# CloudEngineHub/FairyGen

Hardware: AMD Instinct MI355X
Metric: decoded frames/sec (sec/clip in config), Wan2.2-TI2V-5B 704x1280x121 @ 5 steps (higher is better)
Workload: dtype bf16

## Files before the change

### fairygen_amd/csrc/dit_elementwise.hip

```cpp
#include "common.h"
#include "rmsnorm_rope_row.h"

#ifndef FG_ROW_MIN_WAVES
#define FG_ROW_MIN_WAVES 4
#endif
#define FG_ROW_BOUNDS __launch_bounds__(256, FG_ROW_MIN_WAVES)

namespace {

__device__ __forceinline__ void row_moments(const Row& r, int C, int lane, float eps, float& mean, float& rstd) {
    const int nvec = C >> 3;
    float s = 0.f;
#pragma unroll
    for (int i = 0; i < kMaxVec; ++i)
#pragma unroll
        for (int j = 0; j < 8; ++j) s += r.v[i][j];
    mean = wave_sum(s) / (float)C;
    float q = 0.f;
#pragma unroll
    for (int i = 0; i < kMaxVec; ++i) {
        if (lane + i * 64 < nvec) {
#pragma unroll
            for (int j = 0; j < 8; ++j) {
                const float d = r.v[i][j] - mean;
                q += d * d;
            }
        }
    }
    const float var = wave_sum(q) / (float)C;
    rstd = 1.0f / sqrtf(var + eps);
}

__device__ __forceinline__ int64_t mod_row(int64_t row, int64_t mod_rows, int64_t first_rows) {
    return mod_rows == 1 ? 0 : (mod_rows == 2 ? (row < first_rows ? 0 : 1) : row);
}

template <int MODE>
__device__ __forceinline__ void norm_store(const Row& r, int C, int lane, float eps, const bf16* p0, const bf16* p1,
                                           bf16* out) {
    const int nvec = C >> 3;
    float mean, rstd;
    row_moments(r, C, lane, eps, mean, rstd);
#pragma unroll
    for (int i = 0; i < kMaxVec; ++i) {
        const int vi = lane + i * 64;
        if (vi < nvec) {
            const bf16x8 a = ld8(p0 + (int64_t)vi * 8);
            const bf16x8 b = ld8(p1 + (int64_t)vi * 8);
            float o[8];
#pragma unroll
            for (int j = 0; j < 8; ++j) {
                const float n = (r.v[i][j] - mean) * rstd;
                if (MODE == 0) {
                    const float y = rbf(n);
                    const float s1 = rbf(1.0f + (float)b[j]);
                    o[j] = rbf(y * s1) + (float)a[j];
                } else {
                    o[j] = n * (float)a[j] + (float)b[j];
                }
            }
            st8(out + (int64_t)vi * 8, o);
        }
    }
}

__device__ __forceinline__ uint32_t cvt2_fp8(float a, float b) {
    return (uint32_t)__builtin_amdgcn_cvt_pk_fp8_f32(a, b, 0, false) & 0xffffu;
}

template <int MODE, bool DUAL = false>
__device__ __forceinline__ void norm_store_fp8(Row& r, int C, int lane, float eps, const bf16* p0, const bf16* p1,
                                               uint8_t* out8, float* scale_out, float fp8_max, bf16* out16 = nullptr) {
    const int nvec = C >> 3;
    float mean, rstd;
    row_moments(r, C, lane, eps, mean, rstd);
    float amax = 0.f;
#pragma unroll
    for (int i = 0; i < kMaxVec; ++i) {
        const int vi = lane + i * 64;
        if (vi < nvec) {
            const bf16x8 a = ld8(p0 + (int64_t)vi * 8);
            const bf16x8 b = ld8(p1 + (int64_t)vi * 8);
#pragma unroll
            for (int j = 0; j < 8; ++j) {
                const float n = (r.v[i][j] - mean) * rstd;
                float o;
                if (MODE == 0) {
                    const float y = rbf(n);
                    const float s1 = rbf(1.0f + (float)b[j]);
                    o = rbf(y * s1) + (float)a[j];
                } else {
                    o = n * (float)a[j] + (float)b[j];
                }
                r.v[i][j] = rbf(o);
                amax = fmaxf(amax, fabsf(r.v[i][j]));
            }
            if (DUAL) st8(out16 + (int64_t)vi * 8, r.v[i]);
        }
    }
    amax = wave_max(amax);
    const float sc = fmaxf(rbf(amax / fp8_max), 1.0f);
    const float denom = sc + 1e-8f;
    if (lane == 0) *scale_out = sc;
#pragma unroll
    for (int i = 0; i < kMaxVec; ++i) {
        const int vi = lane + i * 64;
        if (vi < nvec) {
            u32x2 w;
            w[0] = cvt2_fp8(r.v[i][0] / denom, r.v[i][1] / denom) | (cvt2_fp8(r.v[i][2] / denom, r.v[i][3] / denom) << 16);
            w[1] = cvt2_fp8(r.v[i][4] / denom, r.v[i][5] / denom) | (cvt2_fp8(r.v[i][6] / denom, r.v[i][7] / denom) << 16);
            *reinterpret_cast<u32x2*>(out8 + (int64_t)vi * 8) = w;
        }
    }
}

__global__ FG_ROW_BOUNDS void ln_modulate_fp8_kernel(const bf16* __restrict__ x, const bf16* __restrict__ shift,
                                                     const bf16* __restrict__ scale, uint8_t* __restrict__ out8,
                                                     float* __restrict__ scale_out, int64_t rows, int C, float eps, int64_t mod_rows,
                                                     int64_t first_rows, int64_t mod_ld, float fp8_max) {
    const int lane = threadIdx.x & 63;
    const int64_t row = (int64_t)blockIdx.x * kRowsPerBlock + (threadIdx.x >> 6);
    if (row >= rows) return;
    Row r;
    load_row(x + row * C, C, lane, r);
    const int64_t m = mod_row(row, mod_rows, first_rows);
    norm_store_fp8<0>(r, C, lane, eps, shift + m * mod_ld, scale + m * mod_ld, out8 + row * C, scale_out + row, fp8_max);
}

template <int MODE>
__global__ FG_ROW_BOUNDS void ln_dual_kernel(const bf16* __restrict__ x, const bf16* __restrict__ p0, const bf16* __restrict__ p1,
                                             bf16* __restrict__ out, uint8_t* __restrict__ out8, float* __restrict__ scale_out,
                                             int64_t rows, int C, float eps, int64_t mod_rows, int64_t first_rows, int64_t mod_ld,
                                             float fp8_max) {
    const int lane = threadIdx.x & 63;
    const int64_t row = (int64_t)blockIdx.x * kRowsPerBlock + (threadIdx.x >> 6);
    if (row >= rows) return;
    Row r;
    load_row(x + row * C, C, lane, r);
    const int64_t m = MODE == 0 ? mod_row(row, mod_rows, first_rows) : 0;
    norm_store_fp8<MODE, true>(r, C, lane, eps, p0 + m * mod_ld, p1 + m * mod_ld, out8 + row * C, scale_out + row, fp8_max, out + row * C);
}

__global__ FG_ROW_BOUNDS void ln_modulate_kernel(const bf16* __restrict__ x, const bf16* __restrict__ shift,
                                                          const bf16* __restrict__ scale, bf16* __restrict__ out,
                                                          int64_t rows, int C, float eps, int64_t mod_rows,
                                                          int64_t first_rows, int64_t mod_ld) {
    const int lane = threadIdx.x & 63;
    const int64_t row = (int64_t)blockIdx.x * kRowsPerBlock + (threadIdx.x >> 6);
    if (row >= rows) return;
    Row r;
    load_row(x + row * C, C, lane, r);
    const int64_t m = mod_row(row, mod_rows, first_rows);
    norm_store<0>(r, C, lane, eps, shift + m * mod_ld, scale + m * mod_ld, out + row * C);
}

__global__ FG_ROW_BOUNDS void ln_affine_kernel(const bf16* __restrict__ x, const bf16* __restrict__ w,
                                                        const bf16* __restrict__ b, bf16* __restrict__ out,
                                                        int64_t rows, int C, float eps) {
    const int lane = threadIdx.x & 63;
    const int64_t row = (int64_t)blockIdx.x * kRowsPerBlock + (threadIdx.x >> 6);
    if (row >= rows) return;
    Row r;
    load_row(x + row * C, C, lane, r);
    norm_store<1>(r, C, lane, eps, w, b, out + row * C);
}

template <int MODE>
__global__ FG_ROW_BOUNDS void residual_kernel(const bf16* __restrict__ x, const bf16* __restrict__ y,
                                                       const bf16* __restrict__ gate, bf16* __restrict__ x_out,
                                                       const bf16* __restrict__ p0, const bf16* __restrict__ p1,
                                                       bf16* __restrict__ norm_out, int64_t rows, int C, float eps,
                                                       int64_t mod_rows, int64_t first_rows, int64_t mod_ld,
                                                       uint8_t* __restrict__ norm_fp8 = nullptr, float* __restrict__ norm_scale = nullptr,
                                                       float fp8_max = 0.f) {
    const int lane = threadIdx.x & 63;
    const int64_t row = (int64_t)blockIdx.x * kRowsPerBlock + (threadIdx.x >> 6);
    if (row >= rows) return;
    const int nvec = C >> 3;
    const int64_t m = mod_row(row, mod_rows, first_rows);
    Row r;
#pragma unroll
    for (int i = 0; i < kMaxVec; ++i) {
        const int vi = lane + i * 64;
        if (vi < nvec) {
            const bf16x8 xv = ld8(x + row * C + (int64_t)vi * 8);
            const bf16x8 yv = ld8(y + row * C + (int64_t)vi * 8);
            if (gate != nullptr) {
                const bf16x8 gv = ld8(gate + m * mod_ld + (int64_t)vi * 8);
#pragma unroll
                for (int j = 0; j < 8; ++j) r.v[i][j] = rbf((float)xv[j] + rbf((float)gv[j] * (float)yv[j]));
            } else {
#pragma unroll
                for (int j = 0; j < 8; ++j) r.v[i][j] = rbf((float)xv[j] + (float)yv[j]);
            }
            st8(x_out + row * C + (int64_t)vi * 8, r.v[i]);
        } else {
#pragma unroll
            for (int j = 0; j < 8; ++j) r.v[i][j] = 0.f;
        }
    }
    if (norm_fp8 != nullptr) {
        if (MODE == 0) norm_store_fp8<0>(r, C, lane, eps, p0 + m * mod_ld, p1 + m * mod_ld, norm_fp8 + row * C, norm_scale + row, fp8_max);
        if (MODE == 1) norm_store_fp8<1>(r, C, lane, eps, p0, p1, norm_fp8 + row * C, norm_scale + row, fp8_max);
        return;
    }
    if (MODE == 0) norm_store<0>(r, C, lane, eps, p0 + m * mod_ld, p1 + m * mod_ld, norm_out + row * C);
    if (MODE == 1) norm_store<1>(r, C, lane, eps, p0, p1, norm_out + row * C);
}

template <bool F32TAB, bool PLAIN = false>
__global__ FG_ROW_BOUNDS void rmsnorm_rope_kernel(const bf16* __restrict__ x, int64_t ldx,
                                                           const bf16* __restrict__ w, const void* __restrict__ ctv,
                                                           const void* __restrict__ stv, bf16* __restrict__ out,
                                                           int64_t rows, int C, int head_dim, float eps, int group_cols,
                                                           int64_t out_group_stride, int64_t out_ld) {
    const int lane = threadIdx.x & 63;
    const int64_t row = (int64_t)blockIdx.x * kRowsPerBlock + (threadIdx.x >> 6);
    if (row >= rows) return;
    Row r;
    load_row(x + row * ldx, C, lane, r);
    const int nvec = C >> 3;
    const RopeRow rr = rope_begin<F32TAB, PLAIN>(r, ctv, row, C, head_dim, eps, lane);
#pragma unroll
    for (int i = 0; i < kMaxVec; ++i) {
        const int vi = lane + i * 64;
        if (vi < nvec) {
            float o[8];
            rope_vec<F32TAB, PLAIN>(rr, r.v[i], ld8(w + (int64_t)vi * 8), ctv, stv, row, head_dim, vi, o);
            const int col = vi * 8, g = PLAIN ? 0 : col / group_cols;
            st8(out + g * out_group_stride + row * out_ld + (col - g * group_cols), o);
        }
    }
}

__global__ __launch_bounds__(256) void copy_groups_kernel(const bf16* __restrict__ src, int64_t sgs, int64_t sld,
                                                          bf16* __restrict__ dst, int64_t dgs, int64_t dld, int groups,
                                                          int64_t rows, int vec_per_row) {
    const int64_t total = (int64_t)groups * rows * vec_per_row;
    for (int64_t i = (int64_t)blockIdx.x * blockDim.x + threadIdx.x; i < total; i += (int64_t)gridDim.x * blockDim.x) {
        const int64_t rg = i / vec_per_row;
        const int v = (int)(i - rg * vec_per_row);
        const int64_t r = rg / groups;
        const int g = (int)(rg - r * groups);
        *reinterpret_cast<u32x4*>(dst + g * dgs + r * dld + v * 8) =
            *reinterpret_cast<const u32x4*>(src + g * sgs + r * sld + v * 8);
    }
}


template <int KIND>
__global__ __launch_bounds__(256) void act_kernel(const bf16* __restrict__ x, bf16* __restrict__ out, int64_t nvec) {
    for (int64_t i = (int64_t)blockIdx.x * blockDim.x + threadIdx.x; i < nvec; i += (int64_t)gridDim.x * blockDim.x) {
        const bf16x8 v = ld8(x + i * 8);
        float o[8];
#pragma unroll
        for (int j = 0; j < 8; ++j) o[j] = KIND == 0 ? silu_f((float)v[j]) : gelu_tanh_f((float)v[j]);
        st8(out + i * 8, o);
    }
}

__device__ __forceinline__ float cfg_euler_one(float lat, float p, float ng, bool has_nega, float cfg, float dsigma) {
    const float pred = has_nega ? rbf(ng + rbf(cfg * rbf(p - ng))) : p;
    return rbf(lat + rbf(pred * dsigma));
}

__global__ __launch_bounds__(256) void cfg_euler_kernel(const bf16* __restrict__ lat, const bf16* __restrict__ posi,
                                                        const bf16* __restrict__ nega, bf16* __restrict__ out,
                                                        int64_t n, float cfg, float dsigma) {
    for (int64_t i = (int64_t)blockIdx.x * blockDim.x + threadIdx.x; i < n; i += (int64_t)gridDim.x * blockDim.x)
        out[i] = (bf16)cfg_euler_one((float)lat[i], (float)posi[i], nega != nullptr ? (float)nega[i] : 0.0f, nega != nullptr, cfg, dsigma);
}

__global__ __launch_bounds__(256) void cfg_euler_dev_kernel(const bf16* lat, const bf16* __restrict__ posi, const bf16* __restrict__ nega,
                                                            bf16* out, int64_t n, int64_t nvec, float cfg,
                                                            const float* __restrict__ dsigma_table, const int* __restrict__ step,
                                                            const bf16* __restrict__ first, int64_t first_n, int64_t frame_stride) {
    const float dsigma = dsigma_table[*step];
    const bool has_nega = nega != nullptr;
    const int64_t tid = (int64_t)blockIdx.x * blockDim.x + threadIdx.x, nthreads = (int64_t)gridDim.x * blockDim.x;
    for (int64_t i = tid; i < nvec; i += nthreads) {
        const bf16x8 l = ld8(lat + i * 8), p = ld8(posi + i * 8);
        const bf16x8 g = has_nega ? ld8(nega + i * 8) : p;
        float o[8];
#pragma unroll
        for (int j = 0; j < 8; ++j) o[j] = cfg_euler_one((float)l[j], (float)p[j], (float)g[j], has_nega, cfg, dsigma);
        if (first != nullptr) {
            int64_t ch = (i * 8) / frame_stride, r = i * 8 - ch * frame_stride;
            if (r < first_n || r + 7 >= frame_stride) {
#pragma unroll
                for (int j = 0; j < 8; ++j) {
                    if (r < first_n) o[j] = (float)first[ch * first_n + r];
                    if (++r == frame_stride) { r = 0; ++ch; }
                }
            }
        }
        st8(out + i * 8, o);
    }
    for (int64_t i = nvec * 8 + tid; i < n; i += nthreads) {
        float o = cfg_euler_one((float)lat[i], (float)posi[i], has_nega ? (float)nega[i] : 0.0f, has_nega, cfg, dsigma);
        if (first != nullptr) {
            const int64_t ch = i / frame_stride, r = i - ch * frame_stride;
            if (r < first_n) o = (float)first[ch * first_n + r];
        }
        out[i] = (bf16)o;
    }
}

inline int check_rows(const char* fn, int64_t rows, int C, int64_t mod_rows, int64_t first_rows) {
    FG_CHECK_ARG(rows >= 0 && C > 0 && (C % 8) == 0 && C <= kMaxVec * 512, "%s: need C %% 8 == 0 and C <= %d (got rows=%lld C=%d)",
                 fn, kMaxVec * 512, (long long)rows, C);
    FG_CHECK_ARG(mod_rows == 1 || mod_rows == 2 || mod_rows == rows, "%s: mod_rows must be 1, 2 or rows (got %lld)", fn,
                 (long long)mod_rows);
    FG_CHECK_ARG(first_rows >= 0 && first_rows <= rows, "%s: first_rows out of range", fn);
    return FG_OK;
}

inline dim3 row_grid(int64_t rows) { return dim3((unsigned)((rows + kRowsPerBlock - 1) / kRowsPerBlock)); }

}

extern "C" {

int fg_ln_modulate_bf16(const void* x, const void* shift, const void* scale, void* out, int64_t rows, int C, float eps,
                        int64_t mod_rows, int64_t first_rows, int64_t mod_ld, fg_stream_t stream) {
    if (int e = check_rows("fg_ln_modulate_bf16", rows, C, mod_rows, first_rows)) return e;
    FG_CHECK_ARG(x && shift && scale && out, "fg_ln_modulate_bf16: null pointer");
    FG_CHECK_ARG(FG_ALIGNED16(x) && FG_ALIGNED16(shift) && FG_ALIGNED16(scale) && FG_ALIGNED16(out) && mod_ld % 8 == 0,
                 "fg_ln_modulate_bf16: pointers / mod_ld must be 16-byte aligned");
    if (rows == 0) return FG_OK;
    hipLaunchKernelGGL(ln_modulate_kernel, row_grid(rows), dim3(256), 0, (hipStream_t)stream, (const bf16*)x,
                       (const bf16*)shift, (const bf16*)scale, (bf16*)out, rows, C, eps, mod_rows, first_rows, mod_ld);
    return fg_launch_status("fg_ln_modulate_bf16");
}

int fg_ln_modulate_fp8_bf16(const void* x, const void* shift, const void* scale, void* out_fp8, float* out_scale, int64_t rows, int C,
                            float eps, int64_t mod_rows, int64_t first_rows, int64_t mod_ld, float fp8_max, fg_stream_t stream) {
    if (int e = check_rows("fg_ln_modulate_fp8_bf16", rows, C, mod_rows, first_rows)) return e;
    FG_CHECK_ARG(x && shift && scale && out_fp8 && out_scale, "fg_ln_modulate_fp8_bf16: null pointer");
    FG_CHECK_ARG(FG_ALIGNED16(x) && FG_ALIGNED16(shift) && FG_ALIGNED16(scale) && (((uintptr_t)out_fp8) & 7) == 0 && mod_ld % 8 == 0 &&
                     fp8_max > 0.f,
                 "fg_ln_modulate_fp8_bf16: pointers / mod_ld must be 16-byte aligned (out_fp8: 8), fp8_max positive");
    if (rows == 0) return FG_OK;
    hipLaunchKernelGGL(ln_modulate_fp8_kernel, row_grid(rows), dim3(256), 0, (hipStream_t)stream, (const bf16*)x, (const bf16*)shift,
                       (const bf16*)scale, (uint8_t*)out_fp8, out_scale, rows, C, eps, mod_rows, first_rows, mod_ld, fp8_max);
    return fg_launch_status("fg_ln_modulate_fp8_bf16");
}

int fg_ln_modulate_dual_bf16(const void* x, const void* shift, const void* scale, void* out, void* out_fp8, float* out_scale,
                             int64_t rows, int C, float eps, int64_t mod_rows, int64_t first_rows, int64_t mod_ld, float fp8_max,
                             fg_stream_t stream) {
    if (int e = check_rows("fg_ln_modulate_dual_bf16", rows, C, mod_rows, first_rows)) return e;
    FG_CHECK_ARG(x && shift && scale && out && out_fp8 && out_scale, "fg_ln_modulate_dual_bf16: null pointer");
    FG_CHECK_ARG(FG_ALIGNED16(x) && FG_ALIGNED16(shift) && FG_ALIGNED16(scale) && FG_ALIGNED16(out) && (((uintptr_t)out_fp8) & 7) == 0 &&
                     mod_ld % 8 == 0 && fp8_max > 0.f,
                 "fg_ln_modulate_dual_bf16: pointers / mod_ld must be 16-byte aligned (out_fp8: 8), fp8_max positive");
    if (rows == 0) return FG_OK;
    hipLaunchKernelGGL(ln_dual_kernel<0>, row_grid(rows), dim3(256), 0, (hipStream_t)stream, (const bf16*)x, (const bf16*)shift,
                       (const bf16*)scale, (bf16*)out, (uint8_t*)out_fp8, out_scale, rows, C, eps, mod_rows, first_rows, mod_ld, fp8_max);
    return fg_launch_status("fg_ln_modulate_dual_bf16");
}

int fg_ln_affine_dual_bf16(const void* x, const void* w, const void* b, void* out, void* out_fp8, float* out_scale, int64_t rows, int C,
                           float eps, float fp8_max, fg_stream_t stream) {
    if (int e = check_rows("fg_ln_affine_dual_bf16", rows, C, 1, 0)) return e;
    FG_CHECK_ARG(x && w && b && out && out_fp8 && out_scale, "fg_ln_affine_dual_bf16: null pointer");
    FG_CHECK_ARG(FG_ALIGNED16(x) && FG_ALIGNED16(w) && FG_ALIGNED16(b) && FG_ALIGNED16(out) && (((uintptr_t)out_fp8) & 7) == 0 &&
                     fp8_max > 0.f,
                 "fg_ln_affine_dual_bf16: pointers must be 16-byte aligned (out_fp8: 8), fp8_max positive");
    if (rows == 0) return FG_OK;
    hipLaunchKernelGGL(ln_dual_kernel<1>, row_grid(rows), dim3(256), 0, (hipStream_t)stream, (const bf16*)x, (const bf16*)w,
                       (const bf16*)b, (bf16*)out, (uint8_t*)out_fp8, out_scale, rows, C, eps, (int64_t)1, (int64_t)0, (int64_t)0, fp8_max);
    return fg_launch_status("fg_ln_affine_dual_bf16");
}

int fg_residual_ln_fp8_bf16(const void* x, const void* y, const void* gate, void* x_out, const void* p0, const void* p1,
                            void* norm_fp8, float* norm_scale, int mode, int64_t rows, int C, float eps, int64_t mod_rows,
                            int64_t first_rows, int64_t mod_ld, float fp8_max, fg_stream_t stream) {
    FG_CHECK_ARG(mode == 0 || mode == 1, "fg_residual_ln_fp8_bf16: mode must be 0 (modulate) or 1 (affine)");
    const bool need_mod = gate != nullptr || mode == 0;
    if (int e = check_rows("fg_residual_ln_fp8_bf16", rows, C, need_mod ? mod_rows : 1, need_mod ? first_rows : 0)) return e;
    FG_CHECK_ARG(x && y && x_out && p0 && p1 && norm_fp8 && norm_scale, "fg_residual_ln_fp8_bf16: null pointer");
    FG_CHECK_ARG(FG_ALIGNED16(x) && FG_ALIGNED16(y) && FG_ALIGNED16(gate) && FG_ALIGNED16(x_out) && FG_ALIGNED16(p0) &&
                     FG_ALIGNED16(p1) && (((uintptr_t)norm_fp8) & 7) == 0 && mod_ld % 8 == 0 && fp8_max > 0.f,
                 "fg_residual_ln_fp8_bf16: pointers / mod_ld must be 16-byte aligned (norm_fp8: 8), fp8_max positive");
    if (rows == 0) return FG_OK;
    if (!need_mod) { mod_rows = 1; first_rows = 0; }
    if (mode == 0)
        hipLaunchKernelGGL(residual_kernel<0>, row_grid(rows), dim3(256), 0, (hipStream_t)stream, (const bf16*)x,
                           (const bf16*)y, (const bf16*)gate, (bf16*)x_out, (const bf16*)p0, (const bf16*)p1,
                           (bf16*)nullptr, rows, C, eps, mod_rows, first_rows, mod_ld, (uint8_t*)norm_fp8, norm_scale, fp8_max);
    else
        hipLaunchKernelGGL(residual_kernel<1>, row_grid(rows), dim3(256), 0, (hipStream_t)stream, (const bf16*)x,
                           (const bf16*)y, (const bf16*)gate, (bf16*)x_out, (const bf16*)p0, (const bf16*)p1,
                           (bf16*)nullptr, rows, C, eps, mod_rows, first_rows, mod_ld, (uint8_t*)norm_fp8, norm_scale, fp8_max);
    return fg_launch_status("fg_residual_ln_fp8_bf16");
}

int fg_ln_affine_bf16(const void* x, const void* w, const void* b, void* out, int64_t rows, int C, float eps,
                      fg_stream_t stream) {
    if (int e = check_rows("fg_ln_affine_bf16", rows, C, 1, 0)) return e;
    FG_CHECK_ARG(x && w && b && out, "fg_ln_affine_bf16: null pointer");
    FG_CHECK_ARG(FG_ALIGNED16(x) && FG_ALIGNED16(w) && FG_ALIGNED16(b) && FG_ALIGNED16(out),
                 "fg_ln_affine_bf16: pointers must be 16-byte aligned");
    if (rows == 0) return FG_OK;
    hipLaunchKernelGGL(ln_affine_kernel, row_grid(rows), dim3(256), 0, (hipStream_t)stream, (const bf16*)x, (const bf16*)w,
                       (const bf16*)b, (bf16*)out, rows, C, eps);
    return fg_launch_status("fg_ln_affine_bf16");
}

int fg_gate_residual_bf16(const void* x, const void* y, const void* gate, void* out, int64_t rows, int C, int64_t mod_rows,
                          int64_t first_rows, int64_t mod_ld, fg_stream_t stream) {
    if (int e = check_rows("fg_gate_residual_bf16", rows, C, gate ? mod_rows : 1, gate ? first_rows : 0)) return e;
    FG_CHECK_ARG(x && y && out, "fg_gate_residual_bf16: null pointer");
    FG_CHECK_ARG(FG_ALIGNED16(x) && FG_ALIGNED16(y) && FG_ALIGNED16(gate) && FG_ALIGNED16(out) && mod_ld % 8 == 0,
                 "fg_gate_residual_bf16: pointers / mod_ld must be 16-byte aligned");
    if (rows == 0) return FG_OK;
    hipLaunchKernelGGL(residual_kernel<-1>, row_grid(rows), dim3(256), 0, (hipStream_t)stream, (const bf16*)x,
                       (const bf16*)y, (const bf16*)gate, (bf16*)out, (const bf16*)nullptr, (const bf16*)nullptr,
                       (bf16*)nullptr, rows, C, 0.f, gate ? mod_rows : 1, gate ? first_rows : 0, mod_ld);
    return fg_launch_status("fg_gate_residual_bf16");
}

int fg_residual_ln_bf16(const void* x, const void* y, const void* gate, void* x_out, const void* p0, const void* p1,
                        void* norm_out, int mode, int64_t rows, int C, float eps, int64_t mod_rows, int64_t first_rows,
                        int64_t mod_ld, fg_stream_t stream) {
    FG_CHECK_ARG(mode == 0 || mode == 1, "fg_residual_ln_bf16: mode must be 0 (modulate) or 1 (affine)");
    const bool need_mod = gate != nullptr || mode == 0;
    if (int e = check_rows("fg_residual_ln_bf16", rows, C, need_mod ? mod_rows : 1, need_mod ? first_rows : 0)) return e;
    FG_CHECK_ARG(x && y && x_out && p0 && p1 && norm_out, "fg_residual_ln_bf16: null pointer");
    FG_CHECK_ARG(FG_ALIGNED16(x) && FG_ALIGNED16(y) && FG_ALIGNED16(gate) && FG_ALIGNED16(x_out) && FG_ALIGNED16(p0) &&
                     FG_ALIGNED16(p1) && FG_ALIGNED16(norm_out) && mod_ld % 8 == 0,
                 "fg_residual_ln_bf16: pointers / mod_ld must be 16-byte aligned");
    if (rows == 0) return FG_OK;
    if (!need_mod) { mod_rows = 1; first_rows = 0; }
    if (mode == 0)
        hipLaunchKernelGGL(residual_kernel<0>, row_grid(rows), dim3(256), 0, (hipStream_t)stream, (const bf16*)x,
                           (const bf16*)y, (const bf16*)gate, (bf16*)x_out, (const bf16*)p0, (const bf16*)p1,
                           (bf16*)norm_out, rows, C, eps, mod_rows, first_rows, mod_ld);
    else
        hipLaunchKernelGGL(residual_kernel<1>, row_grid(rows), dim3(256), 0, (hipStream_t)stream, (const bf16*)x,
                           (const bf16*)y, (const bf16*)gate, (bf16*)x_out, (const bf16*)p0, (const bf16*)p1,
                           (bf16*)norm_out, rows, C, eps, mod_rows, first_rows, mod_ld);
    return fg_launch_status("fg_residual_ln_bf16");
}

int fg_rmsnorm_rope_bf16(const void* x, int64_t ldx, const void* weight, const void* cos_tab, const void* sin_tab,
                         int table_f32, void* out, int64_t rows, int C, int num_heads, float eps, fg_stream_t stream) {
    if (int e = check_rows("fg_rmsnorm_rope_bf16", rows, C, 1, 0)) return e;
    FG_CHECK_ARG(x && weight && out, "fg_rmsnorm_rope_bf16: null pointer");
    FG_CHECK_ARG(table_f32 ? (cos_tab != nullptr && sin_tab == nullptr) : ((cos_tab == nullptr) == (sin_tab == nullptr)),
                 "fg_rmsnorm_rope_bf16: fp64 mode takes both tables or neither, fp32 mode ONE interleaved table in cos_tab");
    FG_CHECK_ARG(num_heads > 0 && C % num_heads == 0 && (C / num_heads) % 8 == 0,
                 "fg_rmsnorm_rope_bf16: head_dim must be a multiple of 8");
    FG_CHECK_ARG(ldx >= C && ldx % 8 == 0 && FG_ALIGNED16(x) && FG_ALIGNED16(weight) && FG_ALIGNED16(out) &&
                     FG_ALIGNED16(cos_tab) && FG_ALIGNED16(sin_tab),
                 "fg_rmsnorm_rope_bf16: pointers / ldx must be 16-byte aligned");
    if (rows == 0) return FG_OK;
    const int hd = C / num_heads;
    const bool plain = (hd & (hd - 1)) == 0;
#define FG_ROPE_LAUNCH(TAB, PL)                                                                                                  \
    hipLaunchKernelGGL((rmsnorm_rope_kernel<TAB, PL>), row_grid(rows), dim3(256), 0, (hipStream_t)stream, (const bf16*)x, ldx,    \
                       (const bf16*)weight, cos_tab, sin_tab, (bf16*)out, rows, C, hd, eps, C, (int64_t)0, (int64_t)C)
    if (table_f32) { if (plain) FG_ROPE_LAUNCH(true, true); else FG_ROPE_LAUNCH(true, false); }
    else { if (plain) FG_ROPE_LAUNCH(false, true); else FG_ROPE_LAUNCH(false, false); }
#undef FG_ROPE_LAUNCH
    return fg_launch_status("fg_rmsnorm_rope_bf16");
}

int fg_rmsnorm_rope_grouped_bf16(const void* x, int64_t ldx, const void* weight, const void* cos_tab,
                                 const void* sin_tab, int table_f32, void* out, int64_t rows, int C, int num_heads, float eps,
                                 int group_cols, int64_t out_group_stride, int64_t out_ld, fg_stream_t stream) {
    if (int e = check_rows("fg_rmsnorm_rope_grouped_bf16", rows, C, 1, 0)) return e;
    FG_CHECK_ARG(x && weight && out, "fg_rmsnorm_rope_grouped_bf16: null pointer");
    FG_CHECK_ARG(table_f32 ? (cos_tab != nullptr && sin_tab == nullptr) : ((cos_tab == nullptr) == (sin_tab == nullptr)),
                 "fg_rmsnorm_rope_grouped_bf16: fp64 mode takes both tables or neither, fp32 mode ONE interleaved table in cos_tab");
    FG_CHECK_ARG(num_heads > 0 && C % num_heads == 0 && (C / num_heads) % 8 == 0,
                 "fg_rmsnorm_rope_grouped_bf16: head_dim must be a multiple of 8");
    FG_CHECK_ARG(group_cols > 0 && group_cols % 8 == 0 && C % group_cols == 0 && out_ld >= group_cols && out_ld % 8 == 0 &&
                     out_group_stride % 8 == 0 && out_group_stride >= 0,
                 "fg_rmsnorm_rope_grouped_bf16: group_cols must divide C; group_cols, out_ld, out_group_stride multiples of 8");
    FG_CHECK_ARG(ldx >= C && ldx % 8 == 0 && FG_ALIGNED16(x) && FG_ALIGNED16(weight) && FG_ALIGNED16(out) &&
                     FG_ALIGNED16(cos_tab) && FG_ALIGNED16(sin_tab),
                 "fg_rmsnorm_rope_grouped_bf16: pointers / ldx must be 16-byte aligned");
    if (rows == 0) return FG_OK;
    if (table_f32)
        hipLaunchKernelGGL((rmsnorm_rope_kernel<true, false>), row_grid(rows), dim3(256), 0, (hipStream_t)stream, (const bf16*)x, ldx,
                           (const bf16*)weight, cos_tab, sin_tab, (bf16*)out, rows, C, C / num_heads, eps, group_cols,
                           out_group_stride, out_ld);
    else
        hipLaunchKernelGGL((rmsnorm_rope_kernel<false, false>), row_grid(rows), dim3(256), 0, (hipStream_t)stream, (const bf16*)x, ldx,
                           (const bf16*)weight, cos_tab, sin_tab, (bf16*)out, rows, C, C / num_heads, eps, group_cols,
                           out_group_stride, out_ld);
    return fg_launch_status("fg_rmsnorm_rope_grouped_bf16");
}

int fg_copy_groups_bf16(const void* src, int64_t src_group_stride, int64_t src_ld, void* dst, int64_t dst_group_stride,
                        int64_t dst_ld, int groups, int64_t rows, int cols, fg_stream_t stream) {
    FG_CHECK_ARG(src && dst, "fg_copy_groups_bf16: null pointer");
    FG_CHECK_ARG(groups > 0 && rows >= 0 && cols > 0 && cols % 8 == 0, "fg_copy_groups_bf16: cols must be a positive multiple of 8");
    FG_CHECK_ARG(src_group_stride % 8 == 0 && src_ld % 8 == 0 && dst_group_stride % 8 == 0 && dst_ld % 8 == 0 &&
                     src_ld >= cols && dst_ld >= cols && FG_ALIGNED16(src) && FG_ALIGNED16(dst),
                 "fg_copy_groups_bf16: strides must be multiples of 8 elements, rows at least cols wide, pointers 16-byte aligned");
    if (rows == 0) return FG_OK;
    const int64_t total = (int64_t)groups * rows * (cols / 8);
    const unsigned grid = (unsigned)((total + 255) / 256 < 16384 ? (total + 255) / 256 : 16384);
    hipLaunchKernelGGL(copy_groups_kernel, dim3(grid), dim3(256), 0, (hipStream_t)stream, (const bf16*)src, src_group_stride,
                       src_ld, (bf16*)dst, dst_group_stride, dst_ld, groups, rows, cols / 8);
    return fg_launch_status("fg_copy_groups_bf16");
}

int fg_act_bf16(const void* x, void* out, int64_t n, int kind, fg_stream_t stream) {
    FG_CHECK_ARG(x && out && n >= 0 && n % 8 == 0, "fg_act_bf16: n must be a multiple of 8");
    FG_CHECK_ARG(kind == 0 || kind == 1, "fg_act_bf16: kind must be 0 (silu) or 1 (gelu_tanh)");
    FG_CHECK_ARG(FG_ALIGNED16(x) && FG_ALIGNED16(out), "fg_act_bf16: pointers must be 16-byte aligned");
    if (n == 0) return FG_OK;
    const int64_t nvec = n / 8;
    const unsigned grid = (unsigned)((nvec + 255) / 256 < 8192 ? (nvec + 255) / 256 : 8192);
    if (kind == 0)
        hipLaunchKernelGGL(act_kernel<0>, dim3(grid), dim3(256), 0, (hipStream_t)stream, (const bf16*)x, (bf16*)out, nvec);
    else
        hipLaunchKernelGGL(act_kernel<1>, dim3(grid), dim3(256), 0, (hipStream_t)stream, (const bf16*)x, (bf16*)out, nvec);
    return fg_launch_status("fg_act_bf16");
}

int fg_cfg_euler_bf16(const void* latents, const void* posi, const void* nega, void* out, int64_t n, float cfg_scale,
                      float dsigma, fg_stream_t stream) {
    FG_CHECK_ARG(latents && posi && out && n >= 0, "fg_cfg_euler_bf16: null pointer");
    if (n == 0) return FG_OK;
    const unsigned grid = (unsigned)((n + 255) / 256 < 4096 ? (n + 255) / 256 : 4096);
    hipLaunchKernelGGL(cfg_euler_kernel, dim3(grid), dim3(256), 0, (hipStream_t)stream, (const bf16*)latents,
                       (const bf16*)posi, (const bf16*)nega, (bf16*)out, n, cfg_scale, dsigma);
    return fg_launch_status("fg_cfg_euler_bf16");
}

int fg_cfg_euler_dev_bf16(const void* latents, const void* posi, const void* nega, void* out, int64_t n, float cfg_scale,
                          const float* dsigma_table, const int* step, const void* first, int64_t first_n, int64_t frame_stride,
                          fg_stream_t stream) {
    FG_CHECK_ARG(latents && posi && out && dsigma_table && step && n >= 0, "fg_cfg_euler_dev_bf16: null pointer");
    FG_CHECK_ARG((((uintptr_t)dsigma_table) & 3) == 0 && (((uintptr_t)step) & 3) == 0, "fg_cfg_euler_dev_bf16: dsigma_table / step must be 4-byte aligned");
    FG_CHECK_ARG(first == nullptr || (first_n > 0 && frame_stride >= first_n && n % frame_stride == 0),
                 "fg_cfg_euler_dev_bf16: with `first`, need 0 < first_n <= frame_stride and n a multiple of frame_stride (got n=%lld first_n=%lld "
                 "frame_stride=%lld)", (long long)n, (long long)first_n, (long long)frame_stride);
    if (n == 0) return FG_OK;
    const bool vec = FG_ALIGNED16(latents) && FG_ALIGNED16(posi) && FG_ALIGNED16(out) && (nega == nullptr || FG_ALIGNED16(nega));
    const int64_t nvec = vec ? n / 8 : 0;
    const int64_t work = nvec > n - nvec * 8 ? nvec : n - nvec * 8;
    const unsigned grid = (unsigned)((work + 255) / 256 < 4096 ? (work + 255) / 256 : 4096);
    hipLaunchKernelGGL(cfg_euler_dev_kernel, dim3(grid), dim3(256), 0, (hipStream_t)stream, (const bf16*)latents, (const bf16*)posi,
                       (const bf16*)nega, (bf16*)out, n, nvec, cfg_scale, dsigma_table, step, (const bf16*)first, first_n, frame_stride);
    return fg_launch_status("fg_cfg_euler_dev_bf16");
}

}
```

### fairygen_amd/csrc/rmsnorm_rope_row.h

```cpp
#pragma once
#include "common.h"

namespace {

constexpr int kMaxVec = 8;
constexpr int kRowsPerBlock = 4;

template <int NV>
struct RowT {
    float v[NV][8];
};
typedef RowT<kMaxVec> Row;

template <int NV>
__device__ __forceinline__ void load_row(const bf16* p, int C, int lane, RowT<NV>& r) {
    const int nvec = C >> 3;
#pragma unroll
    for (int i = 0; i < NV; ++i) {
        const int vi = lane + i * 64;
        if (vi < nvec) {
            bf16x8 t = *reinterpret_cast<const bf16x8*>(p + (int64_t)vi * 8);
#pragma unroll
            for (int j = 0; j < 8; ++j) r.v[i][j] = (float)t[j];
        } else {
#pragma unroll
            for (int j = 0; j < 8; ++j) r.v[i][j] = 0.f;
        }
    }
}

__device__ __forceinline__ bf16x8 ld8(const bf16* p) { return *reinterpret_cast<const bf16x8*>(p); }
__device__ __forceinline__ void st8(bf16* p, const float* f) {
    bf16x8 t;
#pragma unroll
    for (int j = 0; j < 8; ++j) t[j] = (bf16)f[j];
    *reinterpret_cast<bf16x8*>(p) = t;
}

struct RopeRow {
    float rinv;
    bool hoist;
    f32x4 h0, h1;
};

template <bool F32TAB, bool PLAIN, int NV>
__device__ __forceinline__ RopeRow rope_begin(const RowT<NV>& r, const void* ctv, int64_t row, int C, int head_dim, float eps, int lane) {
    RopeRow c;
    float q = 0.f;
#pragma unroll
    for (int i = 0; i < NV; ++i)
#pragma unroll
        for (int j = 0; j < 8; ++j) q += r.v[i][j] * r.v[i][j];
    const float ms = wave_sum(q) / (float)C;
    c.rinv = 1.0f / sqrtf(ms + eps);
    const int half = head_dim >> 1;
    c.hoist = F32TAB && ctv != nullptr && (512 % head_dim) == 0;
    c.h0 = f32x4{0.f, 0.f, 0.f, 0.f};
    c.h1 = f32x4{0.f, 0.f, 0.f, 0.f};
    if (c.hoist) {
        const int d_lane = PLAIN ? ((lane * 8) & (head_dim - 1)) : ((lane * 8) % head_dim);
        const f32x4* tp = reinterpret_cast<const f32x4*>(static_cast<const float*>(ctv) + (row * half + (d_lane >> 1)) * 2);
        c.h0 = tp[0];
        c.h1 = tp[1];
    }
    return c;
}

template <bool F32TAB, bool PLAIN>
__device__ __forceinline__ void rope_vec(const RopeRow& c, const float* rv, const bf16x8 wv, const void* ctv, const void* stv, int64_t row,
                                         int head_dim, int vi, float* o) {
    const int half = head_dim >> 1;
#pragma unroll
    for (int j = 0; j < 8; ++j) o[j] = rbf(rbf(rv[j] * c.rinv) * (float)wv[j]);
    if (ctv != nullptr) {
        const int d0 = PLAIN ? ((vi * 8) & (head_dim - 1)) : ((vi * 8) % head_dim);
        if (F32TAB) {
            f32x4 t0 = c.h0, t1 = c.h1;
            if (!c.hoist) {
                const f32x4* tp = reinterpret_cast<const f32x4*>(static_cast<const float*>(ctv) + (row * half + (d0 >> 1)) * 2);
                t0 = tp[0];
                t1 = tp[1];
            }
            const float cs[8] = {t0[0], t0[1], t0[2], t0[3], t1[0], t1[1], t1[2], t1[3]};
#pragma unroll
            for (int j = 0; j < 4; ++j) {
                const float a = o[2 * j], b = o[2 * j + 1], cc = cs[2 * j], sn = cs[2 * j + 1];
                o[2 * j] = rbf(__builtin_fmaf(a, cc, -(b * sn)));
                o[2 * j + 1] = rbf(__builtin_fmaf(a, sn, b * cc));
            }
        } else {
            const double* cp = static_cast<const double*>(ctv) + row * half + (d0 >> 1);
            const double* sp = static_cast<const double*>(stv) + row * half + (d0 >> 1);
#pragma unroll
            for (int j = 0; j < 4; ++j) {
                const double a = (double)o[2 * j], b = (double)o[2 * j + 1];
                const double cc = cp[j], sn = sp[j];
                o[2 * j] = (float)(bf16)(a * cc - b * sn);
                o[2 * j + 1] = (float)(bf16)(a * sn + b * cc);
            }
        }
    }
}

}
```

Measured before the change: 15.65.

## Persistent grid-stride LN-modulate kernel with LDS-staged tables and prefetched rows

For C=3072 with at most two modulation tables, ln_modulate now launches a capped persistent grid. Each block stages the shift/scale tables into shared memory once, then walks rows in grid stride while prefetching the next row's raw bf16 data into registers. The row arrays are also templated down to 6 vectors instead of 8, which lowers register pressure. The aim is to avoid reloading the modulation tables for every row and to hide global load latency. The cost is a larger LDS footprint and fewer blocks in flight.

```diff
diff --git a/fairygen_amd/csrc/dit_elementwise.hip b/fairygen_amd/csrc/dit_elementwise.hip
--- a/fairygen_amd/csrc/dit_elementwise.hip
+++ b/fairygen_amd/csrc/dit_elementwise.hip
@@ -8,17 +8,18 @@
 
 namespace {
 
-__device__ __forceinline__ void row_moments(const Row& r, int C, int lane, float eps, float& mean, float& rstd) {
+template <int NV>
+__device__ __forceinline__ void row_moments(const RowT<NV>& r, int C, int lane, float eps, float& mean, float& rstd) {
     const int nvec = C >> 3;
     float s = 0.f;
 #pragma unroll
-    for (int i = 0; i < kMaxVec; ++i)
+    for (int i = 0; i < NV; ++i)
 #pragma unroll
         for (int j = 0; j < 8; ++j) s += r.v[i][j];
     mean = wave_sum(s) / (float)C;
     float q = 0.f;
 #pragma unroll
-    for (int i = 0; i < kMaxVec; ++i) {
+    for (int i = 0; i < NV; ++i) {
         if (lane + i * 64 < nvec) {
 #pragma unroll
             for (int j = 0; j < 8; ++j) {
@@ -36,29 +37,32 @@
 }
 
 template <int MODE>
-__device__ __forceinline__ void norm_store(const Row& r, int C, int lane, float eps, const bf16* p0, const bf16* p1,
+__device__ __forceinline__ void norm_vec(const float* rv, float mean, float rstd, const bf16x8 a, const bf16x8 b, float* o) {
+#pragma unroll
+    for (int j = 0; j < 8; ++j) {
+        const float n = (rv[j] - mean) * rstd;
+        if (MODE == 0) {
+            const float y = rbf(n);
+            const float s1 = rbf(1.0f + (float)b[j]);
+            o[j] = rbf(y * s1) + (float)a[j];
+        } else {
+            o[j] = n * (float)a[j] + (float)b[j];
+        }
+    }
+}
+
+template <int MODE, int NV>
+__device__ __forceinline__ void norm_store(const RowT<NV>& r, int C, int lane, float eps, const bf16* p0, const bf16* p1,
                                            bf16* out) {
     const int nvec = C >> 3;
     float mean, rstd;
     row_moments(r, C, lane, eps, mean, rstd);
 #pragma unroll
-    for (int i = 0; i < kMaxVec; ++i) {
+    for (int i = 0; i < NV; ++i) {
         const int vi = lane + i * 64;
         if (vi < nvec) {
-            const bf16x8 a = ld8(p0 + (int64_t)vi * 8);
-            const bf16x8 b = ld8(p1 + (int64_t)vi * 8);
             float o[8];
-#pragma unroll
-            for (int j = 0; j < 8; ++j) {
-                const float n = (r.v[i][j] - mean) * rstd;
-                if (MODE == 0) {
-                    const float y = rbf(n);
-                    const float s1 = rbf(1.0f + (float)b[j]);
-                    o[j] = rbf(y * s1) + (float)a[j];
-                } else {
-                    o[j] = n * (float)a[j] + (float)b[j];
-                }
-            }
+            norm_vec<MODE>(r.v[i], mean, rstd, ld8(p0 + (int64_t)vi * 8), ld8(p1 + (int64_t)vi * 8), o);
             st8(out + (int64_t)vi * 8, o);
         }
     }
@@ -141,17 +145,58 @@
     norm_store_fp8<MODE, true>(r, C, lane, eps, p0 + m * mod_ld, p1 + m * mod_ld, out8 + row * C, scale_out + row, fp8_max, out + row * C);
 }
 
+constexpr int kWalkVec = 6, kWalkC = kWalkVec * 512;
+
+__device__ __forceinline__ void stage_rows(const bf16* __restrict__ p, int64_t ld, int tables, bf16x8* dst) {
+    for (int t = threadIdx.x; t < tables * (kWalkC / 8); t += 256) {
+        const int m = t / (kWalkC / 8), v = t - m * (kWalkC / 8);
+        dst[t] = ld8(p + m * ld + (int64_t)v * 8);
+    }
+}
+
+template <int MODE, int NV, bool PIPE>
+__device__ __forceinline__ void ln_rows(const bf16* __restrict__ x, const bf16* __restrict__ p0, const bf16* __restrict__ p1,
+                                        bf16* __restrict__ out, int64_t rows, int C, float eps, int64_t mod_rows, int64_t first_rows,
+                                        int64_t mod_ld) {
+    const int lane = threadIdx.x & 63;
+    int64_t row = (int64_t)blockIdx.x * kRowsPerBlock + (threadIdx.x >> 6);
+    if (!PIPE) {
+        if (row >= rows) return;
+        RowT<NV> r;
+        load_row(x + row * C, C, lane, r);
+        const int64_t m = MODE == 0 ? mod_row(row, mod_rows, first_rows) : 0;
+        norm_store<MODE>(r, C, lane, eps, p0 + m * mod_ld, p1 + m * mod_ld, out + row * C);
+        return;
+    }
+    static_assert(!PIPE || NV == kWalkVec, "the walk is built for C = 3072");
+    __shared__ bf16x8 tab[PIPE ? 2 * 2 * (kWalkC / 8) : 1];
+    const int tables = MODE == 0 ? (int)mod_rows : 1;
+    stage_rows(p0, mod_ld, tables, tab);
+    stage_rows(p1, mod_ld, tables, tab + 2 * (kWalkC / 8));
+    __syncthreads();
+    if (row >= rows) return;
+    const int64_t W = (int64_t)gridDim.x * kRowsPerBlock;
+    RawRowT<NV> next;
+    issue_row(x + row * kWalkC, kWalkC, lane, next);
+    for (;;) {
+        RowT<NV> r;
+        widen_row(next, kWalkC, lane, r);
+        const int64_t nrow = row + W;
+        if (nrow < rows) issue_row(x + nrow * kWalkC, kWalkC, lane, next);
+        int m = MODE == 0 ? (int)mod_row(row, mod_rows, first_rows) : 0;
+        asm volatile("" : "+v"(m));
+        const bf16* t0 = reinterpret_cast<const bf16*>(tab + m * (kWalkC / 8));
+        norm_store<MODE>(r, kWalkC, lane, eps, t0, t0 + 2 * kWalkC, out + row * kWalkC);
+        if (nrow >= rows) break;
+        row = nrow;
+    }
+}
+
+template <int NV, bool PIPE>
 __global__ FG_ROW_BOUNDS void ln_modulate_kernel(const bf16* __restrict__ x, const bf16* __restrict__ shift,
-                                                          const bf16* __restrict__ scale, bf16* __restrict__ out,
-                                                          int64_t rows, int C, float eps, int64_t mod_rows,
-                                                          int64_t first_rows, int64_t mod_ld) {
-    const int lane = threadIdx.x & 63;
-    const int64_t row = (int64_t)blockIdx.x * kRowsPerBlock + (threadIdx.x >> 6);
-    if (row >= rows) return;
-    Row r;
-    load_row(x + row * C, C, lane, r);
-    const int64_t m = mod_row(row, mod_rows, first_rows);
-    norm_store<0>(r, C, lane, eps, shift + m * mod_ld, scale + m * mod_ld, out + row * C);
+                                                 const bf16* __restrict__ scale, bf16* __restrict__ out, int64_t rows, int C, float eps,
+                                                 int64_t mod_rows, int64_t first_rows, int64_t mod_ld) {
+    ln_rows<0, NV, PIPE>(x, shift, scale, out, rows, C, eps, mod_rows, first_rows, mod_ld);
 }
 
 __global__ FG_ROW_BOUNDS void ln_affine_kernel(const bf16* __restrict__ x, const bf16* __restrict__ w,
@@ -317,6 +362,19 @@
 
 inline dim3 row_grid(int64_t rows) { return dim3((unsigned)((rows + kRowsPerBlock - 1) / kRowsPerBlock)); }
 
+#ifndef FG_ROW_WALK_CAP
+#define FG_ROW_WALK_CAP 1024
+#endif
+inline dim3 row_walk_grid(int64_t rows) {
+    const int64_t g = (rows + kRowsPerBlock - 1) / kRowsPerBlock;
+    return dim3((unsigned)(g < FG_ROW_WALK_CAP ? g : FG_ROW_WALK_CAP));
+}
+#define FG_ROW_WALK(KERNEL, TABLES, ...)                                                                                          \
+    do {                                                                                                                          \
+        if (C == kWalkC && (TABLES) <= 2) hipLaunchKernelGGL((KERNEL<kWalkVec, true>), row_walk_grid(rows), dim3(256), 0, (hipStream_t)stream, __VA_ARGS__); \
+        else hipLaunchKernelGGL((KERNEL<8, false>), row_grid(rows), dim3(256), 0, (hipStream_t)stream, __VA_ARGS__);              \
+    } while (0)
+
 }
 
 extern "C" {
@@ -328,8 +386,8 @@
     FG_CHECK_ARG(FG_ALIGNED16(x) && FG_ALIGNED16(shift) && FG_ALIGNED16(scale) && FG_ALIGNED16(out) && mod_ld % 8 == 0,
                  "fg_ln_modulate_bf16: pointers / mod_ld must be 16-byte aligned");
     if (rows == 0) return FG_OK;
-    hipLaunchKernelGGL(ln_modulate_kernel, row_grid(rows), dim3(256), 0, (hipStream_t)stream, (const bf16*)x,
-                       (const bf16*)shift, (const bf16*)scale, (bf16*)out, rows, C, eps, mod_rows, first_rows, mod_ld);
+    FG_ROW_WALK(ln_modulate_kernel, mod_rows, (const bf16*)x, (const bf16*)shift, (const bf16*)scale, (bf16*)out, rows, C, eps, mod_rows, first_rows,
+                mod_ld);
     return fg_launch_status("fg_ln_modulate_bf16");
 }
 
diff --git a/fairygen_amd/csrc/rmsnorm_rope_row.h b/fairygen_amd/csrc/rmsnorm_rope_row.h
--- a/fairygen_amd/csrc/rmsnorm_rope_row.h
+++ b/fairygen_amd/csrc/rmsnorm_rope_row.h
@@ -11,6 +11,31 @@
     float v[NV][8];
 };
 typedef RowT<kMaxVec> Row;
+
+template <int NV>
+struct RawRowT {
+    bf16x8 v[NV];
+};
+
+template <int NV>
+__device__ __forceinline__ void issue_row(const bf16* p, int C, int lane, RawRowT<NV>& raw) {
+    const int nvec = C >> 3;
+#pragma unroll
+    for (int i = 0; i < NV; ++i) {
+        const int vi = lane + i * 64;
+        raw.v[i] = *reinterpret_cast<const bf16x8*>(p + (int64_t)(vi < nvec ? vi : 0) * 8);
+    }
+}
+template <int NV>
+__device__ __forceinline__ void widen_row(const RawRowT<NV>& raw, int C, int lane, RowT<NV>& r) {
+    const int nvec = C >> 3;
+#pragma unroll
+    for (int i = 0; i < NV; ++i) {
+        const int vi = lane + i * 64;
+#pragma unroll
+        for (int j = 0; j < 8; ++j) r.v[i][j] = vi < nvec ? (float)raw.v[i][j] : 0.f;
+    }
+}
 
 template <int NV>
 __device__ __forceinline__ void load_row(const bf16* p, int C, int lane, RowT<NV>& r) {
```

Measured after the change: 15.69, median of 2. About the same (+0.2%).
